# DevSinghSachan/emdr2

Measured on AMD Instinct MI355X. Metric: mips_queries_per_sec, higher is better.
Workload: dtype f16; 1 GPU; BASELINE configs[1]: MIPS-only top-50, 512 queries/search over a 21015324 x 768 fp16 index resident in HBM; rows=21015324, dim=768, top_k=50, parallelism=index row-sharded x1, all-gather(top-k) + merge, cus=256, allgather_bytes_per_rank=0

## Files before the change

### emdr2_amd/csrc/mips_api.hip

```cpp
#include "../../include/emdr2_mips.h"
#include "mips_kernels.h"
#include "exp_hooks.h"
#include <stdlib.h>

namespace {

#define TIMING_SLOTS 2048
struct Timing {
    bool enabled = false;
    hipEvent_t ev[2 * TIMING_SLOTS] = {};
    int created = 0;
    int n = 0;
    int64_t rows[TIMING_SLOTS] = {};
} g_timing;

int cu_count()
{
    static int cus = 0;
    if (!cus) {
        int dev = 0;
        hipDeviceProp_t prop;
        if (hipGetDevice(&dev) != hipSuccess || hipGetDeviceProperties(&prop, dev) != hipSuccess) return 256;
        cus = prop.multiProcessorCount > 0 ? prop.multiProcessorCount : 256;
    }
// ... 97 lines not shown

static int variant_for(int nq) { return nq <= 128 ? 2 : (nq <= 256 ? 1 : 0); }
static const int kBM[3] = {128, 256, 512};
static const int kBN[3] = {512, 256, 128};

static int search_impl(const void *tiled, int64_t n_rows, int dim, int64_t row_base, const float *emax_sq,
                       const void *queries, int n_q, int k, const int32_t *ids, void *out_dist, int32_t *out_idx,
                       int64_t *out_row, uint32_t *out_flags, void *workspace, size_t workspace_bytes,
                       emdr2_stream_t stream_, int f32, uint4 *out_rec = nullptr, const Shadow *shadow = nullptr)
{
    if (!tiled || !emax_sq || !queries || !out_flags || !workspace) return EMDR2_E_BADARG;
    if (!out_rec && (!out_dist || !out_idx || !out_row)) return EMDR2_E_BADARG;
    if (out_rec && ((uintptr_t)out_rec & 15)) return EMDR2_E_BADARG;
    if (n_q < 1 || k < 1 || k > EMDR2_MAX_TOPK || bad_shape(n_rows, dim) || n_rows < 1) return EMDR2_E_BADARG;
    Workspace w;
    if (carve((char *)workspace, dim, &w) > workspace_bytes) return EMDR2_E_WORKSPACE;
    hipStream_t stream = (hipStream_t)stream_;
    const int kp = k <= 56 ? 64 : 128;
    const int seg0 = env_int("EMDR2_MIPS_SEG0", 8192) / 512 * 512;
    const int growth = env_int("EMDR2_MIPS_GROWTH", 8);
    const int growth_i8 = env_int("EMDR2_MIPS_GROWTH_I8", 2);
    if (seg0 < 512 || seg0 > (int)CAPQ - 512 || growth < 2 || growth_i8 < 2) return EMDR2_E_BADARG;
    const int force_variant = env_int("EMDR2_MIPS_VARIANT", -1);
    const int cus = env_int("EMDR2_MIPS_GRID", cu_count());
    const int scan_kernel = env_int("EMDR2_MIPS_KERNEL", 1);
    const int ablate = env_int("EMDR2_MIPS_ABLATE", 0);

    for (int q0 = 0; q0 < n_q; q0 += EMDR2_MAX_QUERIES_PER_PASS) {
        const int nqp = (n_q - q0) < EMDR2_MAX_QUERIES_PER_PASS ? (n_q - q0) : EMDR2_MAX_QUERIES_PER_PASS;
        int variant = variant_for(nqp);
        if (force_variant >= 0 && force_variant <= 2 && kBN[force_variant] >= nqp) variant = force_variant;
        const int BM = kBM[variant], BN = kBN[variant];
        const uint16_t *qp = (const uint16_t *)queries + (size_t)q0 * dim;
        int rc;
        if ((rc = mips_launch_pack_queries(qp, nqp, dim, BN, w.q_tiled, w.qnorm, stream))) return rc;
        EXP_MIPS_PACK_QUERIES_FRAG(variant, scan_kernel, qp, nqp, dim, w, stream, rc)
        const int64_t dense_rows = n_rows < seg0 ? n_rows : seg0;
        unsigned *const count8 = w.count + 512, *const prog0 = count8 + 8 * 512;
        if ((rc = mips_launch_init(w.tau, w.count, out_flags + q0, BN, nqp, (unsigned)dense_rows, count8,
                                   8 * 512 + (variant == 0 ? 8 * (size_t)SCAN8_PROG_UINTS : 0), stream)))
            return rc;

        ScanParams sp;
        sp.e_tiled = (const char *)tiled;
        sp.q_tiled = w.q_tiled;
        sp.tau = w.tau;
        sp.cand = w.cand;
        sp.count = w.count;
        sp.flags = out_flags + q0;
        sp.dense_out = nullptr;
        sp.nch = dim / 32;
        sp.n_rows = (int)n_rows;
        sp.n_q = nqp;
        sp.capq = CAPQ;
        sp.cand8 = w.cand8;
        sp.count8 = count8;
        sp.dense_row0 = 0;
        sp.tune = env_int("EMDR2_MIPS_TUNE", 17);
        sp.trace = (unsigned long long *)w.cand + (size_t)511 * CAPQ;

        int scan8_launches = 0;
        const bool shadow_ok = shadow && variant <= 1 && scan_kernel == 1 && (dim % 256) == 0 && n_rows - dense_rows >= shadow->min_rows;
        char *const q8_tiled = w.q_frag;
        float *const qc = (float *)(w.q_frag + (size_t)(dim / 64) * 512 * 64);
        if (shadow_ok && (rc = mips_launch_pack_queries_i8(qp, nqp, dim, BN, q8_tiled, qc, stream))) return rc;
        const bool couple = EXP_MIPS_COUPLE();
        int64_t done = 0, seg_end = dense_rows;
        int mode = 1;
        while (done < n_rows) {
            sp.tile_begin = (int)(done / BM);
            sp.tile_end = (int)((seg_end + BM - 1) / BM);
            const int tiles = sp.tile_end - sp.tile_begin;
            const int grid = tiles < cus ? tiles : cus;
            const bool timed = g_timing.enabled && g_timing.n < TIMING_SLOTS;
            if (timed) {
                while (g_timing.created <= g_timing.n) {
                    if (hipEventCreate(&g_timing.ev[2 * g_timing.created]) != hipSuccess ||
                        hipEventCreate(&g_timing.ev[2 * g_timing.created + 1]) != hipSuccess)
                        return EMDR2_E_LAUNCH;
                    ++g_timing.created;
                }
                if (hipEventRecord(g_timing.ev[2 * g_timing.n], stream) != hipSuccess) return EMDR2_E_LAUNCH;
            }
            bool int8_segment = false;
            EXP_MIPS_SCAN_VARIANT(mode, variant, ablate, scan_kernel, sp, w, grid, seg_end, n_rows, done, stream, rc)
            {
                rc = -4;
                if (mode == 0 && variant <= 1 && scan_kernel == 1) {
                    unsigned *prog = (couple && scan8_launches < 8) ? prog0 + (size_t)SCAN8_PROG_UINTS * scan8_launches : nullptr;
                    if (shadow_ok && seg_end - done >= shadow->min_rows) {
                        rc = mips_launch_scan8i(sp, shadow->image, shadow->table, q8_tiled, qc, BN, done, seg_end, cus, prog, stream);
                        if (rc == 0) { int8_segment = true; ++g_shadow_launches; }
                    }
                    if (rc == -4) rc = mips_launch_scan8(sp, BN, done, seg_end, cus, prog, stream);
                    if (rc == 0) ++scan8_launches;
                }
                if (rc == -4) rc = mips_launch_scan(variant, mode, sp, grid, stream);
            }
            if (rc) return rc;
            if (timed) {
                if (hipEventRecord(g_timing.ev[2 * g_timing.n + 1], stream) != hipSuccess) return EMDR2_E_LAUNCH;
                g_timing.rows[g_timing.n] = seg_end - done;
                ++g_timing.n;
            }
            if (int8_segment && (rc = mips_launch_rescore(sp, qp, (unsigned)kp, stream))) return rc;
            if (seg_end < n_rows && (rc = mips_launch_select(w.cand, w.count, w.cand8, count8, w.tau, out_flags + q0, CAPQ, kp, nqp, stream))) return rc;
            done = seg_end;
            const int64_t next_boundary = done * ((shadow_ok && done * (growth_i8 - 1) >= shadow->min_rows) ? growth_i8 : growth);
            seg_end = next_boundary < n_rows ? next_boundary : n_rows;
            if (n_rows - seg_end < seg_end / 2) seg_end = n_rows;
            mode = 0;
        }

        FinalizeParams fp;
        fp.e_tiled = (const char *)tiled;
        fp.queries = qp;
        fp.cand = w.cand;
        fp.count = w.count;
        fp.cand8 = w.cand8;
        fp.count8 = count8;
        fp.tau = w.tau;
        fp.qnorm = w.qnorm;
        fp.emax_sq = emax_sq;
        fp.ids = ids;
        fp.out_rec = out_rec ? out_rec + (size_t)q0 * k : nullptr;
        fp.out_dist = out_rec ? nullptr : (f32 ? (void *)((float *)out_dist + (size_t)q0 * k) : (void *)((uint16_t *)out_dist + (size_t)q0 * k));
        fp.f32 = f32;
        fp.out_idx = out_rec ? nullptr : out_idx + (size_t)q0 * k;
        fp.out_row = out_rec ? nullptr : out_row + (size_t)q0 * k;
        fp.flags = out_flags + q0;
        fp.n_rows = n_rows;
        fp.row_base = row_base;
        fp.dim = dim;
        fp.n_q = nqp;
        fp.k = k;
        fp.kp = kp;
        fp.capq = CAPQ;
        if ((rc = mips_launch_finalize(fp, true, stream))) return rc;
    }
    return EMDR2_OK;
}

int emdr2_mips_search(const void *tiled, int64_t n_rows, int dim, int64_t row_base, const float *emax_sq,
                      const void *queries, int n_q, int k, const int32_t *ids, void *out_dist, int32_t *out_idx,
                      int64_t *out_row, uint32_t *out_flags, void *workspace, size_t workspace_bytes,
                      emdr2_stream_t stream)
{
    return search_impl(tiled, n_rows, dim, row_base, emax_sq, queries, n_q, k, ids, out_dist, out_idx, out_row, out_flags, workspace,
                       workspace_bytes, stream, 0);
}

int emdr2_mips_search_f32(const void *tiled, int64_t n_rows, int dim, int64_t row_base, const float *emax_sq,
                          const void *queries, int n_q, int k, const int32_t *ids, float *out_dist, int32_t *out_idx,
                          int64_t *out_row, uint32_t *out_flags, void *workspace, size_t workspace_bytes,
                          emdr2_stream_t stream)
{
    return search_impl(tiled, n_rows, dim, row_base, emax_sq, queries, n_q, k, ids, out_dist, out_idx, out_row, out_flags, workspace,
                       workspace_bytes, stream, 1);
}

int emdr2_mips_search_records(const void *tiled, int64_t n_rows, int dim, int64_t row_base, const float *emax_sq, const void *queries, int n_q,
                              int k, const int32_t *ids, int f32, void *out_records, uint32_t *out_flags, void *workspace,
                              size_t workspace_bytes, emdr2_stream_t stream)
{
    if (!out_records) return EMDR2_E_BADARG;
    return search_impl(tiled, n_rows, dim, row_base, emax_sq, queries, n_q, k, ids, nullptr, nullptr, nullptr, out_flags, workspace,
                       workspace_bytes, stream, f32 ? 1 : 0, (uint4 *)out_records);
}

int emdr2_mips_shadow_bytes(int64_t n_rows, int dim, size_t *image_bytes, size_t *table_bytes)
{
    if (!image_bytes || !table_bytes || bad_shape(n_rows, dim) || (dim % 256) != 0) return EMDR2_E_BADARG;
    const int64_t padded = (n_rows + 511) / 512 * 512;
    *image_bytes = (size_t)padded * dim;
    *table_bytes = (size_t)(padded / 256) * 4 * sizeof(float);
    return EMDR2_OK;
}

int emdr2_mips_seal_shadow(const void *tiled, int64_t n_rows, int dim, void *shadow, void *table, uint32_t *nonfinite, emdr2_stream_t stream)
{
    if (!tiled || !shadow || !table || !nonfinite || ((uintptr_t)table & 15) || bad_shape(n_rows, dim) || (dim % 256) != 0) return EMDR2_E_BADARG;
    return mips_launch_seal_shadow(tiled, n_rows, dim, shadow, (float *)table, nonfinite, (hipStream_t)stream);
}

int emdr2_mips_search_shadow(const void *tiled, int64_t n_rows, int dim, int64_t row_base, const float *emax_sq, const void *shadow,
                             const void *table, int64_t shadow_min_rows, const void *queries, int n_q, int k, const int32_t *ids, int f32,
                             void *out_dist, int32_t *out_idx, int64_t *out_row, void *out_records, uint32_t *out_flags, void *workspace,
                             size_t workspace_bytes, emdr2_stream_t stream)
// ... 134 lines not shown
```

### emdr2_amd/csrc/mips_kernels.h

```cpp
#pragma once
#include <hip/hip_runtime.h>
#include <stdint.h>

#define CAPQ 16384u
#define SUBCAP 1024u

struct ScanParams {
    const char *e_tiled;
    const char *q_tiled;
    const float *tau;
    uint2 *cand;
    unsigned *count;
    unsigned *flags;
    float *dense_out;
    int nch;
    int tile_begin, tile_end;
    int n_rows;
    int n_q;
    unsigned capq;
    uint2 *cand8;
    unsigned *count8;
    int dense_row0;
    int tune;
    unsigned long long *trace;
};

int mips_launch_scan(int variant, int mode, const ScanParams &p, int grid, hipStream_t stream);
#define SCAN8_PROG_UINTS (256 * 64)
int mips_launch_scan8(const ScanParams &p, int bn, int64_t row_begin, int64_t row_end, int cus, unsigned *prog, hipStream_t stream);
int mips_launch_seal_shadow(const void *tiled, int64_t n_rows, int dim, void *e8, float *blk, unsigned *nonfinite, hipStream_t stream);
int mips_launch_pack_queries_i8(const void *queries, int n_q, int dim, int bn, void *q8_tiled, float *qc, hipStream_t stream);
int mips_launch_scan8i(const ScanParams &p, const void *e8_tiled, const float *blk, const void *q8_tiled, const float *qc, int bn, int64_t row_begin,
                       int64_t row_end, int cus, unsigned *prog, hipStream_t stream);
int mips_launch_rescore(const ScanParams &p, const void *queries, unsigned pre, hipStream_t stream);
int mips_launch_scan_pp(int variant, int depth, const ScanParams &p, int grid, hipStream_t stream);
int mips_launch_scan_q8(int abl, const ScanParams &p, int grid, hipStream_t stream);
int mips_launch_pack_queries_frag(const void *queries, int n_q, int dim, void *q_frag, hipStream_t stream);
int mips_launch_scan_ablate(int abl, const ScanParams &p, int grid, hipStream_t stream);

int mips_launch_pack_rows(const void *rows_rm, int64_t n_chunk, int dim, int64_t row_offset, void *tiled,
                          float *emax_sq, hipStream_t stream);
int mips_launch_unpack_rows(const void *tiled, int dim, const int64_t *row_ids, int64_t n_out, void *rows_rm,
                            hipStream_t stream);
int mips_launch_pack_queries(const void *queries, int n_q, int dim, int bn, void *q_tiled, float *qnorm,
                             hipStream_t stream);
int mips_launch_init(float *tau, unsigned *count, unsigned *flags, int bn, int n_q, unsigned dense_count, unsigned *zero, size_t n_zero,
                     hipStream_t stream);
int mips_launch_select(uint2 *cand, unsigned *count, uint2 *cand8, unsigned *count8, float *tau, unsigned *flags, unsigned capq, int kp, int n_q,
                       hipStream_t stream);
struct FinalizeParams {
    const char *e_tiled;
    const uint16_t *queries;
    const uint2 *cand;
    const unsigned *count;
    uint2 *cand8;
    unsigned *count8;
    const float *tau;
    const float *qnorm;
    const float *emax_sq;
    const int32_t *ids;
    void *out_dist;
    int32_t *out_idx;
    int64_t *out_row;
    unsigned *flags;
    int64_t n_rows, row_base;
    int dim, n_q, k, kp;
    unsigned capq;
    int f32;
    uint4 *out_rec;
};
int mips_launch_finalize(const FinalizeParams &p, bool select_first, hipStream_t stream);
int mips_launch_merge_f32(const float *dist_in, const int32_t *idx_in, const int64_t *row_in, int n_shards, int n_q, int k,
                          float *out_dist, int32_t *out_idx, int64_t *out_row, hipStream_t stream);
int mips_launch_merge_records(const uint4 *rec_in, int n_shards, int n_q, int k, int f32, void *out_dist, int32_t *out_idx, int64_t *out_row,
                              hipStream_t stream);
int mips_launch_pack_records(const void *dist, const int32_t *idx, const int64_t *row, const int32_t *sel, int n_sel, int k, int f32, uint4 *rec,
                             hipStream_t stream);
int mips_launch_merge(const uint16_t *dist_in, const int32_t *idx_in, const int64_t *row_in, int n_shards, int n_q,
                      int k, uint16_t *out_dist, int32_t *out_idx, int64_t *out_row, hipStream_t stream);

int mips_launch_exact_scores(const char *e_tiled, int64_t n_rows, int dim, const uint16_t *queries,
                             const int32_t *sel, int n_sel, uint16_t *hkeys ,
                             hipStream_t stream);
int mips_launch_exact_select(const uint16_t *hkeys, int64_t n_rows, int64_t row_base, const int32_t *sel, int n_sel,
                             int k, const int32_t *ids, uint16_t *out_dist, int32_t *out_idx, int64_t *out_row,
                             unsigned *flags, hipStream_t stream);

int mips_launch_exact_scores_f32(const char *e_tiled, int64_t n_rows, int dim, const uint16_t *queries, const int32_t *sel, int n_sel,
                                 uint32_t *keys , hipStream_t stream);
int mips_launch_exact_select_f32(const uint32_t *keys, int64_t n_rows, int64_t row_base, const int32_t *sel, int n_sel, int k,
                                 const int32_t *ids, float *out_dist, int32_t *out_idx, int64_t *out_row, unsigned *flags, hipStream_t stream);
```

### emdr2_amd/csrc/mips_scan8i.hip

```cpp
#include "mips_device.h"
#include "mips_kernels.h"

namespace {

typedef int intx4 __attribute__((ext_vector_type(4)));

#define S8_BUF 65536
#define S8_SLOT 16384
#define S8_QCAP 2040
#define S8_WCAP 255
#define S8_FLUSH_AT 128

struct Scan8Params {
    ScanParams s;
    int t_begin, t_end;
    int halves;
    int bn;
    int last_stripe;
    int total, per;
    unsigned *prog;
    const float4 *blk;
    const float4 *qc;
};

__device__ __forceinline__ int s8i_theta(float tau, float t, float a, float b, float s, float n, float d)
{
    if (tau == __builtin_inff()) return 0x7fffffff;
    const float ts = t * s;
    if (!(ts > 0.f)) return (int)0x80000000;
    const float eps = (a * n + b * d) * 1.0001f;
    float num = tau - eps;
    num -= fabsf(num) * 1e-6f;
    float x = num * __builtin_amdgcn_rcpf(ts);
    x -= fabsf(x) * 1e-5f;
    x = floorf(x) - 1.f;
    if (!(x > -2.0e9f)) return (int)0x80000000;
    if (x > 2.0e9f) return 0x7fffffff;
    return (int)x;
}

__device__ __forceinline__ void s8_append(const ScanParams &p, unsigned xcc, unsigned q, unsigned score_bits, unsigned row)
{
    const unsigned slot = __hip_atomic_fetch_add(&p.count8[xcc * 512 + q], 1u, __ATOMIC_RELAXED, __HIP_MEMORY_SCOPE_WORKGROUP);
    if (slot < SUBCAP) { p.cand8[((size_t)q * 8 + xcc) * SUBCAP + slot] = make_uint2(score_bits, row); return; }
    const unsigned s2 = __hip_atomic_fetch_add(&p.count[q], 1u, __ATOMIC_RELAXED, __HIP_MEMORY_SCOPE_AGENT);
    if (s2 < p.capq) p.cand[(size_t)q * p.capq + s2] = make_uint2(score_bits, row);
}

__device__ __forceinline__ void s8_flush(const ScanParams &p, const char *qbuf, const unsigned *cnt, int tid, unsigned xcc)
{
    const int region = tid >> 6;
    unsigned m = ((const volatile __attribute__((address_space(3))) unsigned *)cnt)[region];
    if (m > S8_WCAP) m = S8_WCAP;
    for (unsigned i = tid & 63; i < m; i += 64) {
        const uint4 e = ((const uint4 *)qbuf)[region * S8_WCAP + i];
        s8_append(p, xcc, e.z, e.x, e.y);
    }
}

__global__ void __launch_bounds__(512) mips_scan8i_kernel(Scan8Params P)
{
    extern __shared__ __attribute__((aligned(16))) char smem[];
    const ScanParams &p = P.s;
    char *const qbuf = smem + 2 * S8_BUF;
    unsigned *const qcnt = (unsigned *)(qbuf + S8_QCAP * 16);
    const int tid = threadIdx.x, lane = tid & 63;
    const int wave = __builtin_amdgcn_readfirstlane(tid >> 6);
    const int wr = wave >> 2, wc = wave & 3;
    const int l31 = lane & 31, hi = lane >> 5;

    const int xcd = blockIdx.x & 7, slot = blockIdx.x >> 3, wg_per_xcd = gridDim.x >> 3;
    const int seq_lo = xcd * P.per;
    int seq_hi = seq_lo + P.per; if (seq_hi > P.total) seq_hi = P.total;
    const int first = seq_lo + slot;
    if (first >= seq_hi) return;
    const int my_count = (seq_hi - first + wg_per_xcd - 1) / wg_per_xcd;
    const int KT = p.nch >> 1;
    unsigned *const flagw = qcnt + 8;
    if (tid < 8) qcnt[tid] = 0;
    if (tid == 0) *flagw = 0;
    unsigned wq = 0;
    const unsigned xcc = __builtin_amdgcn_s_getreg(20 | (0 << 6) | (3 << 11)) & 7u;
    const int hq = P.halves == 2 ? first & 1 : 0;
    float4 qcv[4];
    float tauv[4];
#pragma unroll
    for (int qt = 0; qt < 4; ++qt) {
        const int q = hq * 256 + wc * 64 + qt * 16 + ((lane & 3) * 4 + ((lane & 15) >> 2));
        tauv[qt] = q < p.n_q ? p.tau[q] : __builtin_inff();
        qcv[qt] = P.qc[q < p.n_q ? q : 0];
    }

    const int ja = (wave >> 2) & 1, qa = wave & 3;
    const int jb = (wave >> 1) & 1, qb = wave & 1;
    const uint32_t offA = (uint32_t)(ja * STRIPE_CHUNK_BYTES + qa * 1024 + lane * 16);
    const uint32_t q_stage = (uint32_t)P.bn * 64;
    const uint32_t offB = (uint32_t)(jb * q_stage + ((wave >> 2) * 64) * 64 + qb * 1024 + lane * 16);
    int s_i = 0, s_kt = 0;
    const char *sA0, *sA1, *sB;
    auto cursor_item = [&](int i) {
        if (i >= my_count) i = my_count - 1;
        const int pos = first + i * wg_per_xcd;
        const int tile = P.t_begin + (P.halves == 2 ? pos >> 1 : pos);
        int st0 = tile * 2, st1 = tile * 2 + 1;
        if (st0 > P.last_stripe) st0 = P.last_stripe;
        if (st1 > P.last_stripe) st1 = P.last_stripe;
        sA0 = p.e_tiled + (size_t)st0 * p.nch * STRIPE_CHUNK_BYTES;
        sA1 = p.e_tiled + (size_t)st1 * p.nch * STRIPE_CHUNK_BYTES;
        sB = p.q_tiled + (size_t)hq * 256 * 64;
    };
    cursor_item(0);
#define S8_STAGE(T, SB)                                                                                                                   \
    do {                                                                                                                                  \
        char *dst_ = smem + (SB) * S8_BUF + (T) * S8_SLOT + wave * 1024;                                                                   \
        if ((T) == 0 || (T) == 3) {                                                                                                       \
            const uint32_t o_ = offA + ((T) == 3 ? 4096 : 0);                                                                             \
            __builtin_amdgcn_global_load_lds((gptr_t *)(sA0 + o_), (lptr_t *)dst_, 16, 0, 0);                                             \
            __builtin_amdgcn_global_load_lds((gptr_t *)(sA1 + o_), (lptr_t *)(dst_ + 8192), 16, 0, 0);                                    \
        } else {                                                                                                                          \
            const uint32_t o_ = offB + ((T) == 2 ? 32 * 64 : 0);                                                                          \
            __builtin_amdgcn_global_load_lds((gptr_t *)(sB + o_), (lptr_t *)dst_, 16, 0, 0);                                              \
            __builtin_amdgcn_global_load_lds((gptr_t *)(sB + o_ + 128 * 64), (lptr_t *)(dst_ + 8192), 16, 0, 0);                          \
        }                                                                                                                                 \
        if ((T) == 3) {                                                                                                                   \
            sA0 += 2 * STRIPE_CHUNK_BYTES; sA1 += 2 * STRIPE_CHUNK_BYTES; sB += 2 * q_stage;                                              \
            if (++s_kt == KT) { s_kt = 0; cursor_item(++s_i); }                                                                           \
        }                                                                                                                                 \
    } while (0)

    const int l15 = lane & 15, lq = lane >> 4;
    const int prow = (l15 & 3) * 4 + (l15 >> 2);
    const int frag_rd = prow * 64 + ((lq ^ ((prow >> 2) & 3)) << 4);
    const int a_rd = wr * 8192 + frag_rd;
    const int b_rd = wc * 4096 + frag_rd;
    intx4 av[2][4], b0v[4], b1v[4];
#define S8_READ_A(BUF, MH)                                                                                                                \
    _Pragma("unroll") for (int c = 0; c < 2; ++c)                                                                                         \
        _Pragma("unroll") for (int rt = 0; rt < 4; ++rt)                                                                                  \
            av[c][rt] = *(const intx4 *)(smem + (BUF) * S8_BUF + ((MH) ? 3 * S8_SLOT : 0) + c * 4096 + rt * 1024 + a_rd)
#define S8_READ_B(BUF, NH, DST)                                                                                                           \
    _Pragma("unroll") for (int c = 0; c < 2; ++c)                                                                                         \
        _Pragma("unroll") for (int ct = 0; ct < 2; ++ct)                                                                                  \
            DST[2 * c + ct] = *(const intx4 *)(smem + (BUF) * S8_BUF + ((NH) ? 2 * S8_SLOT : S8_SLOT) + c * 2048 + ct * 1024 + b_rd)
#define S8_MFMA(MH, NH, BV)                                                                                                               \
    _Pragma("unroll") for (int c = 0; c < 2; ++c)                                                                                         \
        _Pragma("unroll") for (int rt = 0; rt < 4; ++rt)                                                                                  \
            _Pragma("unroll") for (int ct = 0; ct < 2; ++ct)                                                                              \
                acc[4 * (MH) + rt][2 * (NH) + ct] = __builtin_amdgcn_mfma_i32_16x16x64_i8(av[c][rt], BV[2 * c + ct], acc[4 * (MH) + rt][2 * (NH) + ct], 0, 0, 0)
#define S8_MFMA_Z(MH, NH, BV)                                                                                                             \
    _Pragma("unroll") for (int c = 0; c < 2; ++c)                                                                                         \
        _Pragma("unroll") for (int rt = 0; rt < 4; ++rt)                                                                                  \
            _Pragma("unroll") for (int ct = 0; ct < 2; ++ct)                                                                              \
                acc[4 * (MH) + rt][2 * (NH) + ct] = __builtin_amdgcn_mfma_i32_16x16x64_i8(av[c][rt], BV[2 * c + ct], c == 0 ? zero4 : acc[4 * (MH) + rt][2 * (NH) + ct], 0, 0, 0)
#define S8_SYNC_COMPUTE(BETWEEN, MFMAS)                                                                                                   \
    asm volatile("s_waitcnt vmcnt(8)" ::: "memory");                                                                                      \
    __builtin_amdgcn_sched_barrier(0);                                                                                                    \
    __builtin_amdgcn_s_barrier();                                                                                                         \
    __builtin_amdgcn_sched_barrier(0);                                                                                                    \
    BETWEEN;                                                                                                                              \
    __builtin_amdgcn_s_setprio(1);                                                                                                        \
    MFMAS;                                                                                                                                \
    __builtin_amdgcn_s_setprio(0);                                                                                                        \
    __builtin_amdgcn_sched_barrier(0)
#define S8_BARRIER()                                                                                                                      \
    __builtin_amdgcn_s_barrier();                                                                                                         \
    __builtin_amdgcn_sched_barrier(0)
    auto maybe_flush = [&]() {
        unsigned n_ = 0;
#pragma unroll
        for (int w = 0; w < 8; ++w) n_ = max(n_, ((const volatile __attribute__((address_space(3))) unsigned *)qcnt)[w]);
        if (n_ >= S8_FLUSH_AT) {
            s8_flush(p, qbuf, qcnt, tid, xcc);
            asm volatile("s_waitcnt vmcnt(0)" ::: "memory");
            S8_BARRIER();
            if (tid < 8) qcnt[tid] = 0;
            wq = 0;
            S8_BARRIER();
        }
    };
#define S8_MAYBE_FLUSH() maybe_flush()

    unsigned *const prog = (P.prog && P.halves == 2) ? P.prog + (xcd * (wg_per_xcd >> 1) + (slot >> 1)) * 64 : nullptr;
    int ticks = 0;
#define S8_COUPLE()                                                                                                                       \
    if (prog && wave == 0) {                                                                                                              \
        const int tot_ = __builtin_amdgcn_readfirstlane((int)*(volatile __attribute__((address_space(3))) unsigned *)flagw);               \
        if (lane == 0) {                                                                                                                  \
            atomicAdd(prog, 1u);                                                                                                          \
            __builtin_amdgcn_global_load_lds((gptr_t *)prog, (lptr_t *)flagw, 4, 0, 16);         \
        }                                                                                                                                 \
        const int lead_ = 2 * ticks - tot_;                              \
        ++ticks;                                                                                                                          \
        if (!(P.s.tune & 64)) for (int i_ = 0; i_ < (lead_ > 6 ? 6 : lead_) - 1; ++i_) __builtin_amdgcn_s_sleep(16);      \
    }

    intx4 acc[8][4];
    const intx4 zero4 = {0, 0, 0, 0};

    S8_STAGE(0, 0); S8_STAGE(1, 0); S8_STAGE(2, 0); S8_STAGE(3, 0); S8_STAGE(0, 1); S8_STAGE(1, 1);
    asm volatile("s_waitcnt vmcnt(8)" ::: "memory");
    S8_BARRIER();
    if (wr == 1) { S8_BARRIER(); }

    for (int ti = 0; ti < my_count; ++ti) {
#define S8_KPAIR(HOOK, MF)                                                                                                                \
        do {                                                                                                                              \
            S8_READ_B(0, 0, b0v); S8_READ_A(0, 0);                                                                                        \
            __builtin_amdgcn_sched_barrier(0);                                                                                            \
            S8_STAGE(2, 1);                                                                                                               \
            S8_SYNC_COMPUTE(HOOK, MF(0, 0, b0v));                                                                                         \
            S8_BARRIER();                                                                                                                 \
            S8_READ_B(0, 1, b1v);                                                                                                         \
            __builtin_amdgcn_sched_barrier(0);                                                                                            \
            S8_STAGE(3, 1);                                                                                                               \
            S8_SYNC_COMPUTE(, MF(0, 1, b1v));                                                                                             \
            S8_BARRIER();                                                                                                                 \
            S8_READ_A(0, 1);                                                                                                              \
            __builtin_amdgcn_sched_barrier(0);                                                                                            \
            S8_STAGE(0, 0);                                                                                                               \
            S8_SYNC_COMPUTE(, MF(1, 1, b1v));                                                                                             \
            S8_BARRIER();                                                                                                                 \
            S8_STAGE(1, 0);                                                                                                               \
            S8_SYNC_COMPUTE(, MF(1, 0, b0v));                                                                                             \
            S8_BARRIER();                                                                                                                 \
            S8_READ_B(1, 0, b0v); S8_READ_A(1, 0);                                                                                        \
            __builtin_amdgcn_sched_barrier(0);                                                                                            \
            S8_STAGE(2, 0);                                                                                                               \
            S8_SYNC_COMPUTE(, S8_MFMA(0, 0, b0v));                                                                                        \
            S8_BARRIER();                                                                                                                 \
            S8_READ_B(1, 1, b1v);                                                                                                         \
            __builtin_amdgcn_sched_barrier(0);                                                                                            \
            S8_STAGE(3, 0);                                                                                                               \
            S8_SYNC_COMPUTE(, S8_MFMA(0, 1, b1v));                                                                                        \
            S8_BARRIER();                                                                                                                 \
            S8_READ_A(1, 1);                                                                                                              \
            __builtin_amdgcn_sched_barrier(0);                                                                                            \
            S8_STAGE(0, 1);                                                                                                               \
            S8_SYNC_COMPUTE(, S8_MFMA(1, 1, b1v));                                                                                        \
            S8_BARRIER();                                                                                                                 \
            S8_STAGE(1, 1);                                                                                                               \
            S8_SYNC_COMPUTE(, S8_MFMA(1, 0, b0v));                                                                                        \
            S8_COUPLE();                                                                                                                  \
        } while (0)
        S8_KPAIR(if (wr == 0 && ti > 0) S8_MAYBE_FLUSH(), S8_MFMA_Z);
        if (2 < KT) { S8_BARRIER(); }
        for (int kt2 = 2; kt2 < KT; kt2 += 2) {
            S8_KPAIR(, S8_MFMA);
            if (kt2 + 2 < KT) { S8_BARRIER(); }
        }
        if (wr == 0) { S8_BARRIER(); }

        const int pos = first + ti * wg_per_xcd;
        const int tile = P.t_begin + (P.halves == 2 ? pos >> 1 : pos);
        const int elane = (int)__builtin_amdgcn_mbcnt_hi(~0u, __builtin_amdgcn_mbcnt_lo(~0u, 0u));
        const int e15 = elane & 15, eq = elane >> 4;
        const int row_w = tile * 256 + wr * 128 + eq;
        const bool tail = (tile + 1) * 256 > p.n_rows;
        bool stored = false;
        const __attribute__((address_space(4))) float *bk = (const __attribute__((address_space(4))) float *)(uintptr_t)(P.blk + tile);
        const float bs = bk[0], bn_ = bk[1], bd = bk[2];
#pragma unroll
        for (int qt = 0; qt < 4; ++qt) {
            const unsigned q = (unsigned)(hq * 256 + wc * 64 + qt * 16 + (e15 & 3) * 4 + (e15 >> 2));
            const int tau = s8i_theta(tauv[qt], qcv[qt].x, qcv[qt].y, qcv[qt].z, bs, bn_, bd);
            int mr[8];
#pragma unroll
            for (int rt = 0; rt < 8; ++rt) mr[rt] = max(max(acc[rt][qt][0], acc[rt][qt][1]), max(acc[rt][qt][2], acc[rt][qt][3]));
            const int m = max(max(max(mr[0], mr[1]), max(mr[2], mr[3])), max(max(mr[4], mr[5]), max(mr[6], mr[7])));
            if (__builtin_amdgcn_ballot_w64(m >= tau) == 0) continue;
#pragma unroll
            for (int rt = 0; rt < 8; ++rt) {
                if (__builtin_amdgcn_ballot_w64(mr[rt] >= tau) == 0) continue;
#pragma unroll
                for (int r = 0; r < 4; ++r) {
                    const int v = acc[rt][qt][r];
                    const int row = row_w + rt * 16 + 4 * r;
                    const unsigned long long mask = __builtin_amdgcn_ballot_w64((v >= tau) && (!tail || row < p.n_rows));
                    if (mask == 0) continue;
                    if ((mask >> elane) & 1ull) {
                        const unsigned mine = wq + __builtin_amdgcn_mbcnt_hi((unsigned)(mask >> 32), __builtin_amdgcn_mbcnt_lo((unsigned)mask, 0));
                        if (mine < S8_WCAP) {
                            ((uint2 *)qbuf)[2 * (wave * S8_WCAP + mine)] = make_uint2((unsigned)v, (unsigned)row);
                            ((unsigned *)qbuf)[4 * (wave * S8_WCAP + mine) + 2] = q;
                        } else {
                            s8_append(p, xcc, q, (unsigned)v, (unsigned)row);
                            stored = true;
                        }
                    }
                    wq += (unsigned)__popcll(mask);
                }
            }
        }
        if (__builtin_amdgcn_ballot_w64(stored)) asm volatile("s_waitcnt vmcnt(0)" ::: "memory");
        if (wq > S8_WCAP) wq = S8_WCAP;
        if (elane == 0) qcnt[wave] = wq;
        asm volatile("s_waitcnt lgkmcnt(0)" ::: "memory");
        if (wr == 1) {
            S8_BARRIER();
            if (ti + 1 < my_count) S8_MAYBE_FLUSH();
        }
    }
    if (wr == 0) { S8_BARRIER(); }
    if (prog && tid == 0) atomicAdd(prog, 1u << 20);
    asm volatile("s_waitcnt vmcnt(0)" ::: "memory");
    S8_BARRIER();
    s8_flush(p, qbuf, qcnt, tid, xcc);
}

}

namespace {

__device__ __forceinline__ float block_max_256(float v, float *sh)
{
#pragma unroll
    for (int o = 32; o >= 1; o >>= 1) v = fmaxf(v, __shfl_xor(v, o));
    __syncthreads();
    if ((threadIdx.x & 63) == 0) sh[threadIdx.x >> 6] = v;
    __syncthreads();
    return fmaxf(fmaxf(sh[0], sh[1]), fmaxf(sh[2], sh[3]));
}

__device__ __forceinline__ int quant8(float x, float inv)
{
    int v = (int)rintf(x * inv);
    return v > 127 ? 127 : (v < -127 ? -127 : v);
}

__global__ void __launch_bounds__(256) seal_shadow_kernel(const char *__restrict__ tiled, int nch, char *__restrict__ e8, float4 *__restrict__ blk,
                                                          unsigned *__restrict__ nonfinite)
{
    __shared__ float sh[4];
    const int64_t row = (int64_t)blockIdx.x * 256 + threadIdx.x;
    const int nseg = nch * 4;
    float amax = 0.f, n2 = 0.f;
    bool bad = false;
    for (int seg = 0; seg < nseg; ++seg) {
        const uint4 v = *(const uint4 *)(tiled + tiled_seg_offset(row, seg, nch));
        const half8 h = __builtin_bit_cast(half8, v);
#pragma unroll
        for (int j = 0; j < 8; ++j) {
            const float x = (float)h[j];
            bad |= !(fabsf(x) <= 65504.f);
            amax = fmaxf(amax, fabsf(x));
            n2 += x * x;
        }
    }
    if (bad) atomicOr(nonfinite, 1u);
    amax = block_max_256(amax, sh);
    n2 = block_max_256(n2, sh);
    const float s = amax / 127.f;
    const float inv = s > 0.f ? 127.f / amax : 0.f;
    float d2 = 0.f;
    const int nch8 = nch >> 1;
    for (int g = 0; g < nseg / 2; ++g) {
        unsigned w[4];
#pragma unroll
        for (int hf = 0; hf < 2; ++hf) {
            const uint4 v = *(const uint4 *)(tiled + tiled_seg_offset(row, 2 * g + hf, nch));
            const half8 h = __builtin_bit_cast(half8, v);
#pragma unroll
            for (int j = 0; j < 8; j += 4) {
                unsigned pk = 0;
#pragma unroll
                for (int b = 0; b < 4; ++b) {
                    const float x = (float)h[j + b];
                    const int qv = quant8(x, inv);
                    const float r = x - s * (float)qv;
                    d2 += r * r;
                    pk |= ((unsigned)qv & 255u) << (8 * b);
                }
                w[2 * hf + (j >> 2)] = pk;
            }
        }
        *(uint4 *)(e8 + tiled_seg_offset(row, g, nch8)) = make_uint4(w[0], w[1], w[2], w[3]);
    }
    d2 = block_max_256(d2, sh);
    const float nb = sqrtf(n2) * 1.001f;
    if (threadIdx.x == 0) blk[blockIdx.x] = make_float4(s, nb, (sqrtf(d2) + nb * 0x1p-22f) * 1.001f, 0.f);
}

__global__ void pack_queries_i8_kernel(const uint4 *__restrict__ queries, int n_q, int nseg, int bn, char *__restrict__ q8, float4 *__restrict__ qc)
{
    const int q = blockIdx.x, lane = threadIdx.x;
    float amax = 0.f;
    if (q < n_q)
        for (int seg = lane; seg < nseg; seg += 64) {
            const half8 h = __builtin_bit_cast(half8, queries[(size_t)q * nseg + seg]);
#pragma unroll
            for (int j = 0; j < 8; ++j) amax = fmaxf(amax, fabsf((float)h[j]));
        }
#pragma unroll
    for (int o = 32; o >= 1; o >>= 1) amax = fmaxf(amax, __shfl_xor(amax, o));
    const float t = amax / 127.f;
    const float inv = t > 0.f ? 127.f / amax : 0.f;
    float a2 = 0.f, b2 = 0.f;
    for (int g = lane; g < nseg / 2; g += 64) {
        unsigned w[4] = {0u, 0u, 0u, 0u};
        if (q < n_q) {
#pragma unroll
            for (int hf = 0; hf < 2; ++hf) {
                const half8 h = __builtin_bit_cast(half8, queries[(size_t)q * nseg + 2 * g + hf]);
#pragma unroll
                for (int j = 0; j < 8; ++j) {
                    const float x = (float)h[j];
                    const int qv = quant8(x, inv);
                    const float y = t * (float)qv, r = x - y;
                    a2 += r * r; b2 += y * y;
                    w[2 * hf + (j >> 2)] |= ((unsigned)qv & 255u) << (8 * (j & 3));
                }
            }
        }
        const int c = g >> 2, sp = (g & 3) ^ ((q >> 2) & 3);
        *(uint4 *)(q8 + ((size_t)c * bn * 4 + (size_t)q * 4 + sp) * 16) = make_uint4(w[0], w[1], w[2], w[3]);
    }
#pragma unroll
    for (int o = 32; o >= 1; o >>= 1) { a2 += __shfl_xor(a2, o); b2 += __shfl_xor(b2, o); }
    const float ra = sqrtf(a2), rb = sqrtf(b2);
    if (lane == 0) qc[q] = q < n_q ? make_float4(t, (ra + (ra + rb) * 0x1p-22f) * 1.001f, rb * 1.001f, 0.f) : make_float4(0.f, 0.f, 0.f, 0.f);
}

__global__ void __launch_bounds__(256) rescore_kernel(const char *__restrict__ tiled, const uint4 *__restrict__ queries, int nseg, uint2 *cand,
                                                      const unsigned *__restrict__ count, uint2 *cand8, const unsigned *__restrict__ count8,
                                                      unsigned capq, unsigned pre)
{
    const int q = blockIdx.y, list = blockIdx.x, lane = threadIdx.x & 63, wave = threadIdx.x >> 6;
    uint2 *ent;
    unsigned lo, hi;
    if (list < 8) {
        ent = cand8 + ((size_t)q * 8 + list) * SUBCAP; lo = 0; hi = count8[list * 512 + q];
        if (hi > SUBCAP) hi = SUBCAP;
    } else {
        ent = cand + (size_t)q * capq; lo = pre; hi = count[q];
        if (hi > capq) hi = capq;
    }
    const uint4 *qrow = queries + (size_t)q * nseg;
    const int nch = nseg >> 2;
    for (unsigned i0 = lo + 2 * wave; i0 < hi; i0 += 8) {
        const bool two = i0 + 1 < hi;
        const unsigned r0 = ent[i0].y, r1 = ent[two ? i0 + 1 : i0].y;
        float s0 = 0.f, s1 = 0.f;
        for (int seg = lane; seg < nseg; seg += 64) {
            const half8 e0 = __builtin_bit_cast(half8, *(const uint4 *)(tiled + tiled_seg_offset(r0, seg, nch)));
            const half8 e1 = __builtin_bit_cast(half8, *(const uint4 *)(tiled + tiled_seg_offset(r1, seg, nch)));
            const half8 qv = __builtin_bit_cast(half8, qrow[seg]);
#pragma unroll
            for (int j = 0; j < 8; ++j) { s0 += (float)e0[j] * (float)qv[j]; s1 += (float)e1[j] * (float)qv[j]; }
        }
#pragma unroll
        for (int o = 32; o >= 1; o >>= 1) { s0 += __shfl_xor(s0, o); s1 += __shfl_xor(s1, o); }
        if (lane == 0) {
            ent[i0].x = __float_as_uint(s0);
            if (two) ent[i0 + 1].x = __float_as_uint(s1);
        }
    }
}

}

int mips_launch_seal_shadow(const void *tiled, int64_t n_rows, int dim, void *e8, float *blk, unsigned *nonfinite, hipStream_t stream)
{
    const int64_t blocks = (n_rows + 255) / 256;
    if (blocks == 0) return 0;
    hipLaunchKernelGGL(seal_shadow_kernel, dim3((unsigned)blocks), dim3(256), 0, stream, (const char *)tiled, dim / 32, (char *)e8, (float4 *)blk, nonfinite);
    return hipGetLastError() == hipSuccess ? 0 : -3;
}

int mips_launch_pack_queries_i8(const void *queries, int n_q, int dim, int bn, void *q8_tiled, float *qc, hipStream_t stream)
{
    hipLaunchKernelGGL(pack_queries_i8_kernel, dim3(bn), dim3(64), 0, stream, (const uint4 *)queries, n_q, dim / 8, bn, (char *)q8_tiled, (float4 *)qc);
    return hipGetLastError() == hipSuccess ? 0 : -3;
}

int mips_launch_rescore(const ScanParams &p, const void *queries, unsigned pre, hipStream_t stream)
{
    hipLaunchKernelGGL(rescore_kernel, dim3(9, p.n_q), dim3(256), 0, stream, p.e_tiled, (const uint4 *)queries, p.nch * 4, p.cand, p.count, p.cand8,
                       p.count8, p.capq, pre);
    return hipGetLastError() == hipSuccess ? 0 : -3;
}

int mips_launch_scan8i(const ScanParams &p, const void *e8_tiled, const float *blk, const void *q8_tiled, const float *qc, int bn, int64_t row_begin,
                       int64_t row_end, int cus, unsigned *prog, hipStream_t stream)
{
    if ((bn != 256 && bn != 512) || (p.nch & 7) || p.nch < 8 || (row_begin & 255) || row_end <= row_begin || !p.cand8 || !p.count8) return -4;
    Scan8Params P;
    P.s = p;
    P.s.e_tiled = (const char *)e8_tiled;
    P.s.q_tiled = (const char *)q8_tiled;
    P.s.nch = p.nch / 2;
    P.blk = (const float4 *)blk;
    P.qc = (const float4 *)qc;
    P.prog = prog;
    P.bn = bn; P.halves = bn / 256;
    P.t_begin = (int)(row_begin >> 8);
    P.t_end = (int)((row_end + 255) >> 8);
    P.last_stripe = (int)((p.n_rows + STRIPE_ROWS - 1) / STRIPE_ROWS) - 1;
    P.total = (P.t_end - P.t_begin) * P.halves;
    int grid = cus & ~15;
    if (grid < 16) grid = 16;
    if (P.total < grid) return -4;
    P.per = ((P.total + 7) >> 3);
    P.per = (P.per + 1) & ~1;
    constexpr int LDS = 2 * S8_BUF + S8_QCAP * 16 + 128;
    static bool attr_done = false;
    if (!attr_done) {
        if (hipFuncSetAttribute((const void *)mips_scan8i_kernel, hipFuncAttributeMaxDynamicSharedMemorySize, LDS) != hipSuccess) return -3;
        attr_done = true;
    }
    hipLaunchKernelGGL(mips_scan8i_kernel, dim3(grid), dim3(512), LDS, stream, P);
    return hipGetLastError() == hipSuccess ? 0 : -3;
}
```

Before: 61100 queries/s.

## Fuse fp16 rescoring of int8 candidates into the scan8i kernel drain

Removes the separate rescore kernel that recomputed exact fp16 dot products for candidates found by the int8 shadow scan. The scan kernel now computes those scores while draining its LDS candidate queue, using batched readlane-driven fp16 dot products, and drops candidates below tau before appending them. Overflowing candidates are requeued through LDS and scored the same way instead of being appended directly. This saves a kernel launch and a second pass over the candidate lists, and filters appends. In exchange the scan kernel gains register pressure and extra gather traffic and latency inside the scan loop.

```diff
diff --git a/emdr2_amd/csrc/mips_api.hip b/emdr2_amd/csrc/mips_api.hip
--- a/emdr2_amd/csrc/mips_api.hip
+++ b/emdr2_amd/csrc/mips_api.hip
@@ -203,15 +203,14 @@
                 }
                 if (hipEventRecord(g_timing.ev[2 * g_timing.n], stream) != hipSuccess) return EMDR2_E_LAUNCH;
             }
-            bool int8_segment = false;
             EXP_MIPS_SCAN_VARIANT(mode, variant, ablate, scan_kernel, sp, w, grid, seg_end, n_rows, done, stream, rc)
             {
                 rc = -4;
                 if (mode == 0 && variant <= 1 && scan_kernel == 1) {
                     unsigned *prog = (couple && scan8_launches < 8) ? prog0 + (size_t)SCAN8_PROG_UINTS * scan8_launches : nullptr;
                     if (shadow_ok && seg_end - done >= shadow->min_rows) {
-                        rc = mips_launch_scan8i(sp, shadow->image, shadow->table, q8_tiled, qc, BN, done, seg_end, cus, prog, stream);
-                        if (rc == 0) { int8_segment = true; ++g_shadow_launches; }
+                        rc = mips_launch_scan8i(sp, shadow->image, shadow->table, q8_tiled, qc, qp, BN, done, seg_end, cus, prog, stream);
+                        if (rc == 0) ++g_shadow_launches;
                     }
                     if (rc == -4) rc = mips_launch_scan8(sp, BN, done, seg_end, cus, prog, stream);
                     if (rc == 0) ++scan8_launches;
@@ -224,7 +223,6 @@
                 g_timing.rows[g_timing.n] = seg_end - done;
                 ++g_timing.n;
             }
-            if (int8_segment && (rc = mips_launch_rescore(sp, qp, (unsigned)kp, stream))) return rc;
             if (seg_end < n_rows && (rc = mips_launch_select(w.cand, w.count, w.cand8, count8, w.tau, out_flags + q0, CAPQ, kp, nqp, stream))) return rc;
             done = seg_end;
             const int64_t next_boundary = done * ((shadow_ok && done * (growth_i8 - 1) >= shadow->min_rows) ? growth_i8 : growth);
diff --git a/emdr2_amd/csrc/mips_kernels.h b/emdr2_amd/csrc/mips_kernels.h
--- a/emdr2_amd/csrc/mips_kernels.h
+++ b/emdr2_amd/csrc/mips_kernels.h
@@ -30,9 +30,8 @@
 int mips_launch_scan8(const ScanParams &p, int bn, int64_t row_begin, int64_t row_end, int cus, unsigned *prog, hipStream_t stream);
 int mips_launch_seal_shadow(const void *tiled, int64_t n_rows, int dim, void *e8, float *blk, unsigned *nonfinite, hipStream_t stream);
 int mips_launch_pack_queries_i8(const void *queries, int n_q, int dim, int bn, void *q8_tiled, float *qc, hipStream_t stream);
-int mips_launch_scan8i(const ScanParams &p, const void *e8_tiled, const float *blk, const void *q8_tiled, const float *qc, int bn, int64_t row_begin,
-                       int64_t row_end, int cus, unsigned *prog, hipStream_t stream);
-int mips_launch_rescore(const ScanParams &p, const void *queries, unsigned pre, hipStream_t stream);
+int mips_launch_scan8i(const ScanParams &p, const void *e8_tiled, const float *blk, const void *q8_tiled, const float *qc, const void *queries, int bn,
+                       int64_t row_begin, int64_t row_end, int cus, unsigned *prog, hipStream_t stream);
 int mips_launch_scan_pp(int variant, int depth, const ScanParams &p, int grid, hipStream_t stream);
 int mips_launch_scan_q8(int abl, const ScanParams &p, int grid, hipStream_t stream);
 int mips_launch_pack_queries_frag(const void *queries, int n_q, int dim, void *q_frag, hipStream_t stream);
diff --git a/emdr2_amd/csrc/mips_scan8i.hip b/emdr2_amd/csrc/mips_scan8i.hip
--- a/emdr2_amd/csrc/mips_scan8i.hip
+++ b/emdr2_amd/csrc/mips_scan8i.hip
@@ -10,6 +10,8 @@
 #define S8_QCAP 2040
 #define S8_WCAP 255
 #define S8_FLUSH_AT 128
+#define S8_BATCH_FULL 4
+#define S8_BATCH 16
 
 struct Scan8Params {
     ScanParams s;
@@ -21,6 +23,8 @@
     unsigned *prog;
     const float4 *blk;
     const float4 *qc;
+    const char *e16;
+    const uint4 *queries;
 };
 
 __device__ __forceinline__ int s8i_theta(float tau, float t, float a, float b, float s, float n, float d)
@@ -47,15 +51,119 @@
     if (s2 < p.capq) p.cand[(size_t)q * p.capq + s2] = make_uint2(score_bits, row);
 }
 
-__device__ __forceinline__ void s8_flush(const ScanParams &p, const char *qbuf, const unsigned *cnt, int tid, unsigned xcc)
-{
-    const int region = tid >> 6;
-    unsigned m = ((const volatile __attribute__((address_space(3))) unsigned *)cnt)[region];
-    if (m > S8_WCAP) m = S8_WCAP;
-    for (unsigned i = tid & 63; i < m; i += 64) {
-        const uint4 e = ((const uint4 *)qbuf)[region * S8_WCAP + i];
-        s8_append(p, xcc, e.z, e.x, e.y);
-    }
+template <int U>
+__device__ __forceinline__ void s8_score(const char *e16, const uint4 *queries, int nseg, unsigned rowv, unsigned qv, int lane, float (&s)[U])
+{
+    const int nch = nseg >> 2;
+#pragma unroll
+    for (int u = 0; u < U; ++u) s[u] = 0.f;
+    for (int seg = lane; seg < nseg; seg += 64) {
+        asm volatile("" : "+v"(rowv), "+v"(qv));
+        const unsigned loff = (unsigned)((seg >> 2) * 512 + (seg & 3)) * 16u;
+        uint4 ev[U], wv[U];
+#pragma unroll
+        for (int u = 0; u < U; ++u) {
+            const unsigned r = (unsigned)__builtin_amdgcn_readlane((int)rowv, u), ri = r & 127u;
+            ev[u] = *(const uint4 *)(e16 + ((size_t)(r >> 7) * nch * 512 + ri * 4) * 16 + (loff ^ (((ri >> 2) & 3u) << 4)));
+        }
+#pragma unroll
+        for (int u = 0; u < U; ++u) wv[u] = queries[(size_t)(unsigned)__builtin_amdgcn_readlane((int)qv, u) * nseg + seg];
+#pragma unroll
+        for (int u = 0; u < U; ++u) {
+            const half8 e = __builtin_bit_cast(half8, ev[u]), w = __builtin_bit_cast(half8, wv[u]);
+#pragma unroll
+            for (int j = 0; j < 8; ++j) s[u] += (float)e[j] * (float)w[j];
+        }
+    }
+#pragma unroll
+    for (int o = 32; o >= 1; o >>= 1)
+#pragma unroll
+        for (int u = 0; u < U; ++u) s[u] += __shfl_xor(s[u], o);
+}
+
+template <typename T>
+__device__ __forceinline__ T *s8_uniform(T *ptr)
+{
+    const uintptr_t v = (uintptr_t)ptr;
+    return (T *)(((uintptr_t)(unsigned)__builtin_amdgcn_readfirstlane((int)(v >> 32)) << 32) | (unsigned)__builtin_amdgcn_readfirstlane((int)(unsigned)v));
+}
+
+template <int U>
+__device__ __forceinline__ void s8_drain(const char *e16_, const uint4 *queries_, const float *tau_, uint2 *cand8_, unsigned *count8_, uint2 *cand_,
+                                         unsigned *count_, unsigned capq, int nseg, unsigned qbuf_lds, unsigned cnt_lds, int r0, int r1, int all, int wave,
+                                         unsigned xcc)
+{
+    ScanParams p;
+    p.cand8 = s8_uniform(cand8_); p.count8 = s8_uniform(count8_); p.cand = s8_uniform(cand_); p.count = s8_uniform(count_);
+    p.capq = (unsigned)__builtin_amdgcn_readfirstlane((int)capq);
+    const char *const e16 = s8_uniform(e16_);
+    const uint4 *const queries = s8_uniform(queries_);
+    const float *const tau = s8_uniform(tau_);
+    nseg = __builtin_amdgcn_readfirstlane(nseg);
+    r0 = __builtin_amdgcn_readfirstlane(r0); r1 = __builtin_amdgcn_readfirstlane(r1);
+    all = __builtin_amdgcn_readfirstlane(all); wave = __builtin_amdgcn_readfirstlane(wave);
+    xcc = (unsigned)__builtin_amdgcn_readfirstlane((int)xcc);
+    const __attribute__((address_space(3))) intx4 *const qbuf = (const __attribute__((address_space(3))) intx4 *)(uintptr_t)__builtin_amdgcn_readfirstlane((int)qbuf_lds);
+    const volatile __attribute__((address_space(3))) unsigned *const cnt =
+        (const volatile __attribute__((address_space(3))) unsigned *)(uintptr_t)__builtin_amdgcn_readfirstlane((int)cnt_lds);
+    const int lane = (int)__builtin_amdgcn_mbcnt_hi(~0u, __builtin_amdgcn_mbcnt_lo(~0u, 0u));
+    for (int region = r0; region < r1; ++region) {
+        unsigned m = cnt[region];
+        if (m > S8_WCAP) m = S8_WCAP;
+        m = (unsigned)__builtin_amdgcn_readfirstlane((int)m);
+        const unsigned b0 = all ? (unsigned)((wave - region) & 7) : 0u, bstep = all ? 8u : 1u;
+        for (unsigned i0 = b0 * U; i0 < m; i0 += bstep * U) {
+            unsigned i = i0 + (unsigned)(lane & (U - 1));
+            if (i >= m) i = m - 1;
+            const intx4 ent = qbuf[region * S8_WCAP + i];
+            const uint4 mine = make_uint4((unsigned)ent[0], (unsigned)ent[1], (unsigned)ent[2], 0u);
+            const float tq = tau[mine.z];
+            float s[U];
+            s8_score<U>(e16, queries, nseg, mine.y, mine.z, lane, s);
+            float sc = s[0];
+#pragma unroll
+            for (int u = 1; u < U; ++u) sc = lane == u ? s[u] : sc;
+            if (lane < U && i0 + (unsigned)lane < m && !(sc < tq)) s8_append(p, xcc, mine.z, __float_as_uint(sc), mine.y);
+        }
+    }
+    asm volatile("s_waitcnt vmcnt(0)" ::: "memory");
+}
+
+__device__ __forceinline__ unsigned s8_requeue(const char *e16, const uint4 *queries, const float *tau, uint2 *cand8, unsigned *count8, uint2 *cand,
+                                               unsigned *count, unsigned capq, int nseg, unsigned qbuf_lds, unsigned cnt_lds, int wave, unsigned xcc,
+                                               unsigned o0, unsigned o1, unsigned o2, unsigned o3, int row_w, unsigned q0)
+{
+    wave = __builtin_amdgcn_readfirstlane(wave);
+    __attribute__((address_space(3))) unsigned *const qb = (__attribute__((address_space(3))) unsigned *)(uintptr_t)__builtin_amdgcn_readfirstlane((int)qbuf_lds);
+    __attribute__((address_space(3))) unsigned *const cnt = (__attribute__((address_space(3))) unsigned *)(uintptr_t)__builtin_amdgcn_readfirstlane((int)cnt_lds);
+    const int lane = (int)__builtin_amdgcn_mbcnt_hi(~0u, __builtin_amdgcn_mbcnt_lo(~0u, 0u));
+    unsigned over[4] = {o0, o1, o2, o3};
+    unsigned wq = S8_WCAP;
+    for (;;) {
+        if (lane == 0) cnt[wave] = wq;
+        asm volatile("s_waitcnt lgkmcnt(0)" ::: "memory");
+        s8_drain<S8_BATCH_FULL>(e16, queries, tau, cand8, count8, cand, count, capq, nseg, qbuf_lds, cnt_lds, wave, wave + 1, 0, wave, xcc);
+        wq = 0;
+#pragma unroll
+        for (int qt = 0; qt < 4; ++qt) {
+            for (int b = 0; b < 32; ++b) {
+                const bool set = (over[qt] >> b) & 1u;
+                const unsigned long long mask = __builtin_amdgcn_ballot_w64(set);
+                if (mask == 0) continue;
+                const unsigned mine = wq + __builtin_amdgcn_mbcnt_hi((unsigned)(mask >> 32), __builtin_amdgcn_mbcnt_lo((unsigned)mask, 0));
+                if (set && mine < S8_WCAP) {
+                    qb[4 * (wave * S8_WCAP + mine) + 0] = 0u;
+                    qb[4 * (wave * S8_WCAP + mine) + 1] = (unsigned)(row_w + (b >> 2) * 16 + 4 * (b & 3));
+                    qb[4 * (wave * S8_WCAP + mine) + 2] = q0 + 16u * qt;
+                    over[qt] &= ~(1u << b);
+                }
+                wq += (unsigned)__popcll(mask);
+                if (wq > S8_WCAP) wq = S8_WCAP;
+            }
+        }
+        if (__builtin_amdgcn_ballot_w64((over[0] | over[1] | over[2] | over[3]) != 0u) == 0) break;
+    }
+    return wq;
 }
 
 __global__ void __launch_bounds__(512) mips_scan8i_kernel(Scan8Params P)
@@ -165,13 +273,15 @@
 #define S8_BARRIER()                                                                                                                      \
     __builtin_amdgcn_s_barrier();                                                                                                         \
     __builtin_amdgcn_sched_barrier(0)
+#define S8_DRAIN(R0, R1, ALL)                                                                                                             \
+    s8_drain<S8_BATCH>(P.e16, P.queries, p.tau, p.cand8, p.count8, p.cand, p.count, p.capq, p.nch * 8, (unsigned)(uintptr_t)(lptr_t *)qbuf,              \
+             (unsigned)(uintptr_t)(lptr_t *)qcnt, R0, R1, ALL, wave, xcc)
     auto maybe_flush = [&]() {
         unsigned n_ = 0;
 #pragma unroll
         for (int w = 0; w < 8; ++w) n_ = max(n_, ((const volatile __attribute__((address_space(3))) unsigned *)qcnt)[w]);
         if (n_ >= S8_FLUSH_AT) {
-            s8_flush(p, qbuf, qcnt, tid, xcc);
-            asm volatile("s_waitcnt vmcnt(0)" ::: "memory");
+            S8_DRAIN(0, 8, 1);
             S8_BARRIER();
             if (tid < 8) qcnt[tid] = 0;
             wq = 0;
@@ -256,9 +366,9 @@
         const int e15 = elane & 15, eq = elane >> 4;
         const int row_w = tile * 256 + wr * 128 + eq;
         const bool tail = (tile + 1) * 256 > p.n_rows;
-        bool stored = false;
         const __attribute__((address_space(4))) float *bk = (const __attribute__((address_space(4))) float *)(uintptr_t)(P.blk + tile);
         const float bs = bk[0], bn_ = bk[1], bd = bk[2];
+        unsigned over[4] = {0u, 0u, 0u, 0u};
 #pragma unroll
         for (int qt = 0; qt < 4; ++qt) {
             const unsigned q = (unsigned)(hq * 256 + wc * 64 + qt * 16 + (e15 & 3) * 4 + (e15 >> 2));
@@ -283,16 +393,19 @@
                             ((uint2 *)qbuf)[2 * (wave * S8_WCAP + mine)] = make_uint2((unsigned)v, (unsigned)row);
                             ((unsigned *)qbuf)[4 * (wave * S8_WCAP + mine) + 2] = q;
                         } else {
-                            s8_append(p, xcc, q, (unsigned)v, (unsigned)row);
-                            stored = true;
+                            over[qt] |= 1u << (4 * rt + r);
                         }
                     }
                     wq += (unsigned)__popcll(mask);
                 }
             }
         }
-        if (__builtin_amdgcn_ballot_w64(stored)) asm volatile("s_waitcnt vmcnt(0)" ::: "memory");
         if (wq > S8_WCAP) wq = S8_WCAP;
+        if (__builtin_amdgcn_ballot_w64((over[0] | over[1] | over[2] | over[3]) != 0u))
+            wq = (unsigned)__builtin_amdgcn_readfirstlane((int)s8_requeue(
+                P.e16, P.queries, p.tau, p.cand8, p.count8, p.cand, p.count, p.capq, p.nch * 8, (unsigned)(uintptr_t)(lptr_t *)qbuf,
+                (unsigned)(uintptr_t)(lptr_t *)qcnt, wave, xcc, over[0], over[1], over[2], over[3], row_w,
+                (unsigned)(hq * 256 + wc * 64 + (e15 & 3) * 4 + (e15 >> 2))));
         if (elane == 0) qcnt[wave] = wq;
         asm volatile("s_waitcnt lgkmcnt(0)" ::: "memory");
         if (wr == 1) {
@@ -304,7 +417,7 @@
     if (prog && tid == 0) atomicAdd(prog, 1u << 20);
     asm volatile("s_waitcnt vmcnt(0)" ::: "memory");
     S8_BARRIER();
-    s8_flush(p, qbuf, qcnt, tid, xcc);
+    S8_DRAIN(0, 8, 1);
 }
 
 }
@@ -420,42 +533,6 @@
     if (lane == 0) qc[q] = q < n_q ? make_float4(t, (ra + (ra + rb) * 0x1p-22f) * 1.001f, rb * 1.001f, 0.f) : make_float4(0.f, 0.f, 0.f, 0.f);
 }
 
-__global__ void __launch_bounds__(256) rescore_kernel(const char *__restrict__ tiled, const uint4 *__restrict__ queries, int nseg, uint2 *cand,
-                                                      const unsigned *__restrict__ count, uint2 *cand8, const unsigned *__restrict__ count8,
-                                                      unsigned capq, unsigned pre)
-{
-    const int q = blockIdx.y, list = blockIdx.x, lane = threadIdx.x & 63, wave = threadIdx.x >> 6;
-    uint2 *ent;
-    unsigned lo, hi;
-    if (list < 8) {
-        ent = cand8 + ((size_t)q * 8 + list) * SUBCAP; lo = 0; hi = count8[list * 512 + q];
-        if (hi > SUBCAP) hi = SUBCAP;
-    } else {
-        ent = cand + (size_t)q * capq; lo = pre; hi = count[q];
-        if (hi > capq) hi = capq;
-    }
-    const uint4 *qrow = queries + (size_t)q * nseg;
-    const int nch = nseg >> 2;
-    for (unsigned i0 = lo + 2 * wave; i0 < hi; i0 += 8) {
-        const bool two = i0 + 1 < hi;
-        const unsigned r0 = ent[i0].y, r1 = ent[two ? i0 + 1 : i0].y;
-        float s0 = 0.f, s1 = 0.f;
-        for (int seg = lane; seg < nseg; seg += 64) {
-            const half8 e0 = __builtin_bit_cast(half8, *(const uint4 *)(tiled + tiled_seg_offset(r0, seg, nch)));
-            const half8 e1 = __builtin_bit_cast(half8, *(const uint4 *)(tiled + tiled_seg_offset(r1, seg, nch)));
-            const half8 qv = __builtin_bit_cast(half8, qrow[seg]);
-#pragma unroll
-            for (int j = 0; j < 8; ++j) { s0 += (float)e0[j] * (float)qv[j]; s1 += (float)e1[j] * (float)qv[j]; }
-        }
-#pragma unroll
-        for (int o = 32; o >= 1; o >>= 1) { s0 += __shfl_xor(s0, o); s1 += __shfl_xor(s1, o); }
-        if (lane == 0) {
-            ent[i0].x = __float_as_uint(s0);
-            if (two) ent[i0 + 1].x = __float_as_uint(s1);
-        }
-    }
-}
-
 }
 
 int mips_launch_seal_shadow(const void *tiled, int64_t n_rows, int dim, void *e8, float *blk, unsigned *nonfinite, hipStream_t stream)
@@ -472,19 +549,15 @@
     return hipGetLastError() == hipSuccess ? 0 : -3;
 }
 
-int mips_launch_rescore(const ScanParams &p, const void *queries, unsigned pre, hipStream_t stream)
-{
-    hipLaunchKernelGGL(rescore_kernel, dim3(9, p.n_q), dim3(256), 0, stream, p.e_tiled, (const uint4 *)queries, p.nch * 4, p.cand, p.count, p.cand8,
-                       p.count8, p.capq, pre);
-    return hipGetLastError() == hipSuccess ? 0 : -3;
-}
-
-int mips_launch_scan8i(const ScanParams &p, const void *e8_tiled, const float *blk, const void *q8_tiled, const float *qc, int bn, int64_t row_begin,
-                       int64_t row_end, int cus, unsigned *prog, hipStream_t stream)
+int mips_launch_scan8i(const ScanParams &p, const void *e8_tiled, const float *blk, const void *q8_tiled, const float *qc, const void *queries, int bn,
+                       int64_t row_begin, int64_t row_end, int cus, unsigned *prog, hipStream_t stream)
 {
     if ((bn != 256 && bn != 512) || (p.nch & 7) || p.nch < 8 || (row_begin & 255) || row_end <= row_begin || !p.cand8 || !p.count8) return -4;
+    if (!queries || ((uintptr_t)queries & 15)) return -4;
     Scan8Params P;
     P.s = p;
+    P.e16 = p.e_tiled;
+    P.queries = (const uint4 *)queries;
     P.s.e_tiled = (const char *)e8_tiled;
     P.s.q_tiled = (const char *)q8_tiled;
     P.s.nch = p.nch / 2;
```

Result: slower. 59300 queries/s (-2.9%).
